# jqnfxa/Simplex-Method-Solver

Hardware: AMD Instinct MI355X
Metric: pivots/sec + achieved HBM GB/s, dense fp64 tableau, 1/2/4/8 MI355X (higher is better)
Workload: dtype f64; 1 GPU; 16384x16384 dense fp64 tableau, uniform random LP seed 0; rows=16384, cols=16384, n=16383, m=16383, parallelism=single GPU

## Files before the change

### simplex-method-solver_amd/csrc/smx_block.hpp

```cpp
#pragma once
#pragma clang fp contract(off)

namespace {

template <bool B>
struct SmxBool {
    static constexpr bool value = B;
};

constexpr int kBlkMax = 24;
constexpr int kBlkSlots = kBlkMax + 2;
constexpr int kBlkNT = kUpdBlock;
constexpr int kBlkScan = 4 * kBlkNT;
constexpr int kBlkPartsPer = kUpdBlock / kBlkNT;
constexpr int kBlkPartsMax = 4 * kMaxParts * kBlkPartsPer;
__host__ __device__ __forceinline__ int blk_parts_of(int nparts, int rows) {
    const int by_rows = (rows + kBlkNT - 1) / kBlkNT;
    int g = nparts * kBlkPartsPer;
    if (by_rows > g) g = by_rows;
    return g < kBlkPartsMax ? g : kBlkPartsMax;
}

struct BlkHdr {
    int32_t peff;
// ... 937 lines not shown
        int P, int parity, int bn, smx_ctl* __restrict__ ctl, BlkHdr* __restrict__ h,              \
        smx_part* __restrict__ parts, double* __restrict__ mul, double* __restrict__ pr,           \
        double* __restrict__ fr, const double* __restrict__ recv, int nranks,                      \
        int32_t* __restrict__ log, double* __restrict__ xhist, int64_t log_cap,                    \
        const double* __restrict__ xrow, int64_t xslot
#define SMX_BLK_STEP_ARGS                                                                           \
    T, ld, rows, m, flen, fscan, row0, P, parity, bn, ctl, h, parts, mul, pr, fr, recv, nranks,     \
        log, xhist, log_cap, xrow, xslot

template <int L, bool SH>
__global__ __launch_bounds__(kBlkNT) void k_blk_step(SMX_BLK_STEP_PARAMS) {
    blk_step_body<L, SH>(SMX_BLK_STEP_ARGS);
}

#undef SMX_BLK_STEP_PARAMS
#undef SMX_BLK_STEP_ARGS


template <int P, class PRS>
__device__ __forceinline__ dbl2 blk_exact_h(dbl2 v, int row, int j, const BlkHdr* __restrict__ h,
                                            const double* eq, PRS prs, const double* pc) {
#pragma unroll
    for (int q = 0; q < P; ++q) {
        const int rq = h->r[q], cq = h->c[q];
        const dbl2 p = prs(q);
#pragma unroll
        for (int hh = 0; hh < 2; ++hh) {
            const int jj = j + hh;
            double num;
            if (row == rq) {
                num = (jj == cq) ? 1.0 : -v[hh];
            } else {
                const double a = v[hh] * eq[q];
                const double b = p[hh] * pc[q];
                num = (jj == cq) ? v[hh] : (a - b);
            }
            v[hh] = num / eq[q];
        }
    }
    return v;
}

enum : int {
    kPcFast = 0,
    kPcZero,
    kPcWindow,
    kPcWindowFail,
    kPcExact,
    kPcChunkNotFree,
    kPcChunkNotZok,
    kPcRowFlag0,
    kPcRowFlag3,
    kPcXFail,
    kPcChunkE,
    kPcChunkP,
    kPcClkCycles,
    kPcClkTicks,
    kPcCount
};
#ifdef SMX_PATH_COUNT
__device__ unsigned long long g_path_cnt[kPcCount];
#define SMX_PC_DECL                                                                             \
    uint64_t pc_cnt[kPcCount] = {};                                                             \
    const uint64_t pc_t0 = __builtin_amdgcn_s_memtime();                                        \
    const uint64_t pc_r0 = __builtin_amdgcn_s_memrealtime();
#define SMX_PC(k) (++pc_cnt[(k)])
#define SMX_PC_FLUSH                                                                            \
    do {                                                                                        \
        pc_cnt[kPcClkCycles] = __builtin_amdgcn_s_memtime() - pc_t0;                            \
        pc_cnt[kPcClkTicks] = __builtin_amdgcn_s_memrealtime() - pc_r0;                         \
        const int l_ = threadIdx.x & (kWave - 1);                                               \
        uint64_t v_ = 0;                                                                        \
        _Pragma("unroll") for (int k_ = 0; k_ < kPcCount; ++k_) if (l_ == k_) v_ = pc_cnt[k_];  \
        if (l_ < kPcCount && v_) atomicAdd(&g_path_cnt[l_], (unsigned long long)v_);            \
    } while (0)
#else
#define SMX_PC_DECL
#define SMX_PC(k) ((void)0)
#define SMX_PC_FLUSH ((void)0)
#endif

__device__ int g_sweep_items = 16;

template <int P, int FORM>
__device__ __forceinline__ void blk_sweep_body_flag(const double* Tin, double* Tout, int64_t ld,
                                                    int R, int C, const BlkHdr* __restrict__ h,
                                                    const double* __restrict__ pr,
                                                    const double* __restrict__ mul) {
    constexpr bool LDS = FORM >= 5;
    constexpr bool ITEMS = FORM == 6;
    __shared__ dbl2 s_pr[LDS ? P : 1][kWave];
    __shared__ dbl2 s_ey[LDS ? P : 1];
    __shared__ dbl2 s_zm[LDS ? P : 1];
    __shared__ double s_zf;
    const int32_t* __restrict__ rfl = blk_rflags(mul, R);
    const int lane = threadIdx.x & (kWave - 1);
    const int wib = __builtin_amdgcn_readfirstlane(threadIdx.x >> 6);
    double eq[LDS ? 1 : P], yq[LDS ? 1 : P];
    bool allok = true;
#pragma unroll
    for (int q = 0; q < P; ++q) allok = allok && h->ok[q] != 0;
    constexpr int kChunk = 2 * kWave;
    const int nchunks = (C + kChunk - 1) / kChunk;
    int ch, base, qs;
    int c0 = 0, K = 1, stride = 1, seg = R;
    if constexpr (LDS) {
        ch = (int)blockIdx.x % nchunks;
        base = ((int)blockIdx.x / nchunks) * kUpdWaves + wib;
        qs = ((int)gridDim.x / nchunks) * kUpdWaves;
        if constexpr (ITEMS) {
            c0 = ch;
            K = max(1, min(g_sweep_items, nchunks));
            stride = max(1, nchunks / K);
            seg = ((R + K - 1) / K + qs - 1) / qs * qs;
        }
    } else {
        const int NW = (int)gridDim.x * kUpdWaves;
        const int w = (int)blockIdx.x * kUpdWaves + wib;
        ch = w % nchunks;
        base = w / nchunks;
        qs = NW / nchunks;
    }
    int j = ch * kChunk + 2 * lane;
    dbl2 prs[LDS ? 1 : P];
    auto stage = [&]() {
        for (int t = threadIdx.x; t < P * kWave; t += kUpdBlock) {
            const int q = t / kWave, jl = ch * kChunk + 2 * (t % kWave);
            s_pr[q][t % kWave] = jl < C ? *reinterpret_cast<const dbl2*>(pr + (int64_t)q * ld + jl)
                                        : dbl2{0.0, 0.0};
        }
    };
    if constexpr (LDS) {
        stage();
        if (threadIdx.x < P) {
            const int q = threadIdx.x;
            const double e = h->e[q];
            s_ey[q] = dbl2{e, h->y[q]};
            const double M = q == 0 ? e : (h->e[q - 1] < 0.0 ? e : -e);
            s_zm[q] = dbl2{M, fabs(h->y[q])};
            if (q == P - 1) s_zf = e < 0.0 ? 1.0 : -1.0;
        }
        __syncthreads();
    } else {
#pragma unroll
        for (int q = 0; q < P; ++q) {
            eq[q] = h->e[q];
            yq[q] = h->y[q];
            prs[q] = (j < C) ? *reinterpret_cast<const dbl2*>(pr + (int64_t)q * ld + j)
                             : dbl2{0.0, 0.0};
        }
    }
    auto PR = [&](int q) -> dbl2 {
        if constexpr (LDS) return s_pr[q][lane];
        else return prs[q];
    };
    auto EY = [&](int q) -> dbl2 {
        if constexpr (LDS) return s_ey[q];
        else return dbl2{eq[q], yq[q]};
    };
    const bool kNoFree = g_blk_nofree != 0;
    SMX_PC_DECL
    bool chunk_zok, chunk_free;
    auto chunk_flags = [&]() {
        uint32_t et = 0, pt = 0;
        bool zok = true;
#pragma unroll
        for (int q = 0; q < P; ++q) {
            const dbl2 p = PR(q);
            et = max(et, bnd_term(EY(q)[0]));
            if (j < C) {
                pt = max(pt, bnd_term(p[0]));
                zok = zok && bnd_or_zero(p[0]);
            }
// ... 75 lines not shown
                        const double tq = n[k] * y;
                        const double r = fma(-e, tq, n[k]);
                        rr[k] = fma(r, y, tq);
                    }
                    v0 = dbl2{rr[0], rr[1]};
                }
            }
            ok = true;
        } else if (chunk_zok && (rf & 1) && __all(bnd_or_zero(x0[0]) && bnd_or_zero(x0[1]))) {
            asm volatile("" ::: "memory");
            SMX_PC(kPcZero);
            if constexpr (!LDS) {
                dbl2 bq[P];
#pragma unroll
                for (int q = 0; q < P; ++q)
                    bq[q] = dbl2{prs[q][0] * pc0[q], prs[q][1] * pc0[q]};
#pragma unroll
                for (int q = 0; q < P; ++q) asm volatile("" : "+v"(bq[q]));
#pragma unroll
                for (int q = 0; q < P; ++q) {
                    const double e = eq[q], y = yq[q];
                    const double n0 = v0[0] * e - bq[q][0];
                    const double n1 = v0[1] * e - bq[q][1];
                    v0 = dbl2{fd_zero(n0, e, y), fd_zero(n1, e, y)};
                }
            } else {
#pragma unroll
                for (int q = 0; q < P && !SMX_ZNEG; ++q) {
                    const dbl2 p = PR(q);
                    const dbl2 ey = EY(q);
                    const double e = ey[0], y = ey[1];
                    double n[2];
                    n[0] = v0[0] * e - p[0] * pc0[q];
                    n[1] = v0[1] * e - p[1] * pc0[q];
                    v0 = dbl2{fd_zero(n[0], e, y), fd_zero(n[1], e, y)};
                }
#pragma unroll
                for (int q = 0; q < P && SMX_ZNEG; ++q) {
                    const dbl2 p = PR(q);
                    const dbl2 my = s_zm[q];
                    const double M = my[0], ya = my[1];
                    double n[2];
                    n[0] = v0[0] * M - p[0] * pc0[q];
                    n[1] = v0[1] * M - p[1] * pc0[q];
                    v0 = dbl2{fd_zneg(n[0], fabs(M), ya), fd_zneg(n[1], fabs(M), ya)};
                }
            }
            if (LDS && SMX_ZNEG) v0 = dbl2{v0[0] * s_zf, v0[1] * s_zf};
            ok = true;
        } else if (allok && rf != 2) {
            uint32_t wt = 0;
#pragma unroll
            for (int q = 0; q < P; ++q) {
                const dbl2 p = PR(q);
                const dbl2 ey = EY(q);
                const double e = ey[0], y = ey[1];
                double n[2];
                n[0] = v0[0] * e - p[0] * pc0[q];
                n[1] = v0[1] * e - p[1] * pc0[q];
                double rr[2];
#pragma unroll
                for (int k = 0; k < 2; ++k) {
                    const uint32_t tk = win_term(n[k]);
                    wt = max(wt, (dbits(n[k]) << 1) == 0 ? 0u : tk);
                    rr[k] = fd_zero(n[k], e, y);
                }
                v0 = dbl2{rr[0], rr[1]};
            }
            ok = __all(wt < kWinSpan);
            SMX_PC(ok ? kPcWindow : kPcWindowFail);
        } else {
            SMX_PC(kPcExact);
        }
        if (!ok) {
            x0 = ldc(i0);
            asm volatile("s_waitcnt vmcnt(0)" : "+v"(x0) :: "memory");
#pragma unroll
            for (int q = 0; q < P; ++q) eqa[q] = h->e[q];
            v0 = blk_exact_h<P>(x0, i0, j, h, eqa, PR, pc0);
        }
        if (j < C)
            __builtin_nontemporal_store(v0, reinterpret_cast<dbl2*>(Tout + (int64_t)i0 * ld + j));
    };
    if constexpr (!ITEMS) {
        if (base >= R) return;
    }
    for (int it = 0; it < K; ++it) {
        int lo = 0, hi = R;
        if constexpr (ITEMS) {
            lo = it * seg;
            hi = min(R, lo + seg);
            if (it > 0) {
                ch = (c0 + it * stride) % nchunks;
                j = ch * kChunk + 2 * lane;
                jc = min(j, (C - 1) & ~1);
                __syncthreads();
                stage();
                __syncthreads();
                chunk_flags();
            }
            if (lo + base >= hi) continue;
        }
        const int r0 = lo + base;
        dbl2 a = ldc(r0), b = ldc(r0 + qs);
        asm volatile("s_waitcnt vmcnt(1)" : "+v"(a) :: "memory");
        for (int i0 = r0; i0 < hi; i0 += 2 * qs) {
            rowf(a, i0);
            if (i0 + qs >= hi) break;
            a = ldc(i0 + 2 * qs);
            asm volatile("s_waitcnt vmcnt(2)" : "+v"(b) :: "memory");
            rowf(b, i0 + qs);
            if (i0 + 2 * qs >= hi) break;
            b = ldc(i0 + 3 * qs);
            asm volatile("s_waitcnt vmcnt(2)" : "+v"(a) :: "memory");
        }
        asm volatile("s_waitcnt vmcnt(0)" ::: "memory");
    }
    SMX_PC_FLUSH;
}

__device__ __forceinline__ void blk_fixcols(double* out, int64_t ld, int R, int P,
                                            const BlkHdr* __restrict__ h,
                                            const double* __restrict__ mul,
                                            const double* __restrict__ pr) {
    const double* mT = blk_mulT(mul, R);
    const int64_t pairs = (int64_t)R * P;
    for (int64_t t = (int64_t)blockIdx.x * kUpdBlock + threadIdx.x; t < pairs;
         t += (int64_t)gridDim.x * kUpdBlock) {
        const int q = (int)(t / R), i = (int)(t % R);
        const int c = h->c[q];
        bool last = true;
        for (int q2 = q + 1; q2 < P; ++q2) last = last && h->c[q2] != c;
        if (!last) continue;
        const double* mr = mul + (int64_t)i * kBlkMax;
        const bool frow = i == R - 1;
        double mq[kBlkMax], pc[kBlkMax], eq[kBlkMax];
        int rq[kBlkMax];
#pragma unroll
        for (int q2 = 0; q2 < kBlkMax; ++q2) {
            const bool act = q2 >= q && q2 < P;
            mq[q2] = act ? (frow ? mr[q2] : mT[(int64_t)q2 * R + i]) : 0.0;
            pc[q2] = (act && q2 > q) ? pr[(int64_t)q2 * ld + c] : 0.0;
            eq[q2] = act ? h->e[q2] : 1.0;
            rq[q2] = act ? h->r[q2] : -1;
        }
        double x = 0.0;
#pragma unroll
        for (int q2 = 0; q2 < kBlkMax; ++q2) {
            if (q2 < q || q2 >= P) continue;
            double num;
            if (q2 == q)
                num = (i == rq[q2]) ? 1.0 : mq[q2];
            else if (i == rq[q2])
                num = -x;
            else
                num = x * eq[q2] - pc[q2] * mq[q2];
            x = num / eq[q2];
        }
        out[(int64_t)i * ld + c] = x;
    }
}

__device__ __forceinline__ double* blk_out(double* b_in, double* b_other, int ipx, int in_idx,
                                           int applied, BlkHdr* __restrict__ hs) {
    const bool inplace = ipx >= 0 && ((ipx + applied) & 1) == 0;
    if (blockIdx.x == 0 && threadIdx.x == 0) hs->loc = inplace ? in_idx : in_idx ^ 1;
    return inplace ? b_in : b_other;
}

template <int P, int FORM>
__global__ __launch_bounds__(kUpdBlock) void k_blk_sweep(double* b_in, double* b_other, int64_t ld,
                                                         int R, int C,
                                                         const BlkHdr* __restrict__ h,
                                                         const double* __restrict__ mul,
                                                         const double* __restrict__ pr,
                                                         BlkHdr* __restrict__ hs, int ipx,
                                                         int in_idx) {
    if (h->peff != P) return;
    double* out = blk_out(b_in, b_other, ipx, in_idx, P, hs);
    blk_sweep_body_flag<P, FORM>(b_in, out, ld, R, C, h, pr, mul);
}

__device__ __forceinline__ void blk_publish_wave(const BlkHdr* __restrict__ h,
                                                 const smx_part* __restrict__ parts, int nparts,
                                                 int slot, int parity, smx_ctl* __restrict__ ctl) {
    if (ctl->term) return;
// ... 70 lines not shown
```

### simplex-method-solver_amd/csrc/smx_kernels.hip

```cpp
#include <hip/hip_runtime.h>

#include <math.h>
#include <stddef.h>
#include <stdint.h>
#include <stdio.h>
#include <stdlib.h>
#include <mutex>
#include <thread>
#include <vector>
#include <type_traits>
#include <utility>
#include <string.h>

#include <rccl/rccl.h>

#include "smx.h"

#pragma clang fp contract(off)

static_assert(sizeof(smx_ctl) == 128, "smx_ctl layout");
static_assert(offsetof(smx_ctl, term) == 16 && offsetof(smx_ctl, npivots) == 40 &&
                  offsetof(smx_ctl, shard_off) == 56 && offsetof(smx_ctl, xpos) == 64 &&
                  offsetof(smx_ctl, npiv) == 80 && offsetof(smx_ctl, dec) == 96,
              "smx_ctl offsets (mirrored in simplex_mi355x/_lib.py)");
// ... 307 lines not shown
                       reinterpret_cast<uint64_t*>(xch + p.row_off), s.ld, epoch,
                       g_resident_trace, g_resident_trace_from,
                       reinterpret_cast<uint64_t*>(xch + p.pc_off));
    return (int)hipGetLastError();
}

int resident_serialize(hipStream_t st, bool after) {
    static std::mutex mu;
    static hipEvent_t last[64] = {};
    int dev = 0;
    if (hipStreamGetDevice(st, &dev) != hipSuccess) (void)hipGetDevice(&dev);
    if (dev < 0 || dev >= 64) return (int)hipErrorInvalidDevice;
    std::lock_guard<std::mutex> lock(mu);
    if (!last[dev]) {
        int cur = 0;
        (void)hipGetDevice(&cur);
        hipError_t e = hipSetDevice(dev);
        if (e == hipSuccess) e = hipEventCreateWithFlags(&last[dev], hipEventDisableTiming);
        (void)hipSetDevice(cur);
        if (e != hipSuccess) return (int)e;
        if (!after) return 0;
    }
    return (int)(after ? hipEventRecord(last[dev], st) : hipStreamWaitEvent(st, last[dev], 0));
}

int launch_resident(double* buf0, double* buf1, const smx_shape& s, int parity, int k,
                    smx_ctl* ctl, void* xch, int64_t xch_bytes, uint32_t epoch, int32_t* log,
                    double* xhist, int64_t log_cap, hipStream_t st) {
    ResPlan p;
    if (!resident_plan(s, &p) || xch == nullptr || xch_bytes < p.bytes || epoch < 1 ||
        epoch > 4095 || k >= (1 << 20) - 1)
        return (int)hipErrorInvalidValue;
    hipError_t e = hipMemsetAsync(&ctl->dec[0][0], 0, sizeof(int32_t), st);
    if (e != hipSuccess) return (int)e;
    int err = resident_serialize(st, false);
    if (!err)
        err = launch_resident_kernel(buf0, buf1, s, p, parity, k, ctl, static_cast<char*>(xch),
                                     epoch, log, xhist, log_cap, st);
    if (!err) err = resident_serialize(st, true);
    return err;
}

int g_block = 0;
constexpr int64_t kBlockMinTable = 48ll << 20;
constexpr int64_t kBlockWideTable = 256ll << 20;

constexpr int64_t kBlockHugeTable = 1ll << 30;
bool wplan_shape(const smx_shape& s);

int block_pivots(const smx_shape& s) {
    if (g_block == 1) return 0;
    if (s.row0 != 0 || s.rows != s.n || s.rows < 1 || s.m < 1) return 0;
    if (g_block >= 2) return g_block;
    const int64_t bytes = (int64_t)(s.rows + 1) * s.ld * 8;
    if (bytes < kBlockMinTable) return 0;
    if (wplan_shape(s)) return kBlkMax;
    if (bytes >= kBlockHugeTable) return 20;
    return bytes >= kBlockWideTable ? 12 : 10;
}

int block_size(int k, int P, int b) {
    const int nb = (k + P - 1) / P;
    const int base = k / nb, extra = k % nb;
    return base + (b < extra ? 1 : 0);
}

using BlkSweepFn = void (*)(double*, double*, int64_t, int, int, const BlkHdr*, const double*,
                           const double*, BlkHdr*, int, int);
using BlkStepFn = void (*)(const double*, int64_t, int, int, int, int, int, int, int, int,
                           smx_ctl*, BlkHdr*, smx_part*, double*, double*, double*,
                           const double*, int, int32_t*, double*, int64_t, const double*,
                           int64_t);
using BshPackFn = void (*)(const double*, int64_t, int, int, int, int, int, const smx_ctl*,
                           const BlkHdr*, const smx_part*, int, const double*, const double*,
                           double*);

template <int FORM, int... Is>
BlkSweepFn blk_sweep_pick(int P, std::integer_sequence<int, Is...>) {
    static const BlkSweepFn t[] = {k_blk_sweep<Is + 1, FORM>...};
    return t[P - 1];
}
BlkSweepFn blk_sweep_fn(int P, int form) {
    using All = std::make_integer_sequence<int, kBlkMax>;
    return form == 6 ? blk_sweep_pick<6>(P, All{})
                     : form == 5 ? blk_sweep_pick<5>(P, All{}) : blk_sweep_pick<4>(P, All{});
}

template <bool SH, int... Is>
BlkStepFn blk_step_pick(int L, std::integer_sequence<int, Is...>) {
    static const BlkStepFn t[] = {k_blk_step<Is + 1, SH>...};
    return t[L - 1];
}
template <bool SH>
BlkStepFn blk_step_fn_sh(int L) {
    return blk_step_pick<SH>(L, std::make_integer_sequence<int, kBlkMax>{});
}

template <int... Is>
BshPackFn bsh_pack_pick(int D, std::integer_sequence<int, Is...>) {
    static const BshPackFn t[] = {k_bsh_pack<Is>...};
    return t[D];
}
BshPackFn bsh_pack_fn(int D) { return bsh_pack_pick(D, std::make_integer_sequence<int, kBlkMax>{}); }

struct BlkPtrs {
    BlkLayout L;
    BlkHdr* h[2];
    smx_part* parts;
    double *mul[2], *pr[2], *fr, *win;
    uint64_t* xg;
};
int g_block_planner = 0;
int g_block_nwin = kWin;
bool use_window(const smx_shape& s, bool sh) {
    return !sh && g_block_planner != 1 && s.row0 == 0 && s.rows == s.n;
}
bool use_wplan(const smx_shape& s, bool sh) {
    return use_window(s, sh) && g_block_planner == 0 && win_rpw(s.rows) <= kWpMaxRpw &&
           win_groups(s.rows) <= num_cus();
}
bool wplan_shape(const smx_shape& s) { return use_wplan(s, false); }

int blk_G(const smx_shape& s, bool sh) {
    return use_window(s, sh) ? win_groups(s.rows) : blk_parts_of(s.nparts, s.rows);
}

BlkPtrs blk_ptrs(const smx_shape& s, char* blk) {
    BlkPtrs b;
    b.L = blk_layout(s.rows + 1, s.ld, blk_parts_of(s.nparts, s.rows));
    for (int k = 0; k < 2; ++k) {
        b.h[k] = reinterpret_cast<BlkHdr*>(blk + kBlkHdrBytes * k);
        b.mul[k] = reinterpret_cast<double*>(blk + b.L.mul + k * b.L.mul_slot);
        b.pr[k] = reinterpret_cast<double*>(blk + b.L.pr + k * b.L.pr_slot);
    }
    b.parts = reinterpret_cast<smx_part*>(blk + b.L.parts);
    b.fr = reinterpret_cast<double*>(blk + b.L.fr);
    b.win = reinterpret_cast<double*>(blk + b.L.win);
    b.xg = reinterpret_cast<uint64_t*>(blk + b.L.xg);
    return b;
}

int launch_blk_prime(bool sh, const double* T, const smx_shape& s, int parity, int loc, smx_ctl* ctl,
                     const BlkPtrs& b, hipStream_t st) {
    hipLaunchKernelGGL(k_blk_start, dim3(blk_G(s, sh)), dim3(kBlkNT), 0, st, T, s.ld, s.rows, s.m,
                       fscan_of(s), parity, loc, s.row0, (const smx_ctl*)ctl, b.h[0], b.h[1],
                       b.fr, b.parts, use_wplan(s, sh) ? b.xg : nullptr);
    return (int)hipGetLastError();
}

int launch_blk_step(bool sh, int L, const double* T, const smx_shape& s, int P, int parity,
                    int bn, smx_ctl* ctl, const BlkPtrs& b, const double* recv, int nranks,
                    int32_t* log, double* xhist, int64_t log_cap, hipStream_t st,
                    const double* xrow = nullptr, int64_t xslot = 0) {
    BlkStepFn fn = sh ? blk_step_fn_sh<true>(L) : blk_step_fn_sh<false>(L);
    hipLaunchKernelGGL(fn, dim3(blk_G(s, sh)), dim3(kBlkNT), 0, st, T, s.ld, s.rows, s.m, s.flen,
                       fscan_of(s), s.row0, P, parity, bn, ctl, b.h[0], b.parts, b.mul[0],
                       b.pr[0], b.fr, recv, nranks, log, xhist, log_cap, xrow, xslot);
    return (int)hipGetLastError();
}

int launch_blk_wplan(const double* T, const smx_shape& s, int P, int parity, int bn, int done,
                     smx_ctl* ctl, const BlkPtrs& b, int32_t* log, double* xhist,
                     int64_t log_cap, hipStream_t st) {
    hipLaunchKernelGGL(k_blk_wplan, dim3(win_groups(s.rows)), dim3(kWinNT), 0, st, T, s.ld,
                       s.rows, s.m, s.flen, fscan_of(s), P, parity, bn, done, g_block_nwin,
                       win_rpw(s.rows), ctl, b.h[0], b.parts, b.mul[0], b.pr[0], b.xg, log,
                       xhist, log_cap);
    return (int)hipGetLastError();
}

int launch_blk_wstep(int L, const double* T, const smx_shape& s, int P, int parity, int bn,
                     smx_ctl* ctl, const BlkPtrs& b, int32_t* log, double* xhist, int64_t log_cap,
                     hipStream_t st, int fromT) {
    hipLaunchKernelGGL(k_blk_wstep, dim3(win_groups(s.rows)), dim3(kWinNT), 0, st, T, s.ld,
                       s.rows, s.m, s.flen, fscan_of(s), P, L, parity, bn, g_block_nwin,
                       win_rpw(s.rows), fromT, ctl, b.h[0], b.parts, b.mul[0], b.win, log, xhist,
                       log_cap);
    return (int)hipGetLastError();
}
int launch_blk_prows(const double* T, const smx_shape& s, int P, const BlkPtrs& b,
                     hipStream_t st) {
    const int64_t work = std::max<int64_t>((int64_t)(s.m + 1) * 4, s.rows + 1);
    const int grid = (int)std::min<int64_t>((work + kProwsNT - 1) / kProwsNT, num_cus() * 8);
    hipLaunchKernelGGL(k_blk_prows, dim3(grid), dim3(kProwsNT), 0, st, T, s.ld, s.rows, s.m, P,
                       (const BlkHdr*)b.h[0], b.mul[0], b.pr[0]);
    return (int)hipGetLastError();
}

int g_shard_xchg = -1;
bool xchg_light(int nranks) { return g_shard_xchg < 0 ? nranks >= 4 : g_shard_xchg == 1; }

int launch_bsh_pick(const double* hdrs, const smx_shape& s, int nranks, int rank,
                    const double* send, double* row, hipStream_t st) {
    const int grid = (int)((s.ld + kUpdBlock - 1) / kUpdBlock);
    hipLaunchKernelGGL(k_bsh_pick, dim3(grid < 1 ? 1 : grid), dim3(kUpdBlock), 0, st, hdrs,
                       nranks, s.ld, s.m, s.flen, rank, send, row);
    return (int)hipGetLastError();
}

int launch_bsh_pack(int D, const double* T, const smx_shape& s, int P, int bn,
                    const smx_ctl* ctl, const BlkPtrs& b, double* send, hipStream_t st) {
    const int gc = (int)std::min<int64_t>((s.m + 1 + kBlkNT - 1) / kBlkNT, kBlkPartsMax);
    const int grid = std::max(blk_parts_of(s.nparts, s.rows), gc);
    hipLaunchKernelGGL(bsh_pack_fn(D), dim3(grid), dim3(kBlkNT), 0, st, T, s.ld, s.rows,
                       s.m, s.row0, P, bn, ctl, (const BlkHdr*)b.h[0], (const smx_part*)b.parts,
                       blk_parts_of(s.nparts, s.rows), (const double*)b.mul[0], (const double*)b.pr[0], send);
    return (int)hipGetLastError();
}

int launch_blk_publish(bool sh, const smx_shape& s, int parity, int bn, smx_ctl* ctl, const BlkPtrs& b,
                       hipStream_t st) {
    hipLaunchKernelGGL(k_blk_publish, dim3(1), dim3(kWave), 0, st, (const BlkHdr*)b.h[0],
                       (const smx_part*)b.parts, blk_G(s, sh), blk_slot(0, 1, bn), parity, ctl);
    return (int)hipGetLastError();
}

int g_block_form = 0;
constexpr int kSweepRegMaxP = 12;
constexpr int64_t kSweepItemRows = 2048;

int sweep_grid_lds(const smx_shape& s, int bpc) {
    const int64_t nchunks = (s.m + 1 + 2 * kWave - 1) / (2 * kWave);
    int64_t per = (int64_t)num_cus() * bpc / nchunks;
    const int64_t rows_per = (s.rows + 1 + kUpdWaves - 1) / kUpdWaves;
    if (per > rows_per) per = rows_per;
    if (per < 1) per = 1;
    return (int)(per * nchunks);
}

int launch_block_sweep(bool sh, double* tin, double* tother, const smx_shape& s, int P, char* blk,
                       const BlkLayout& L, hipStream_t st, int slot = 0, int ipx = 0,
                       int in_idx = 0, int ipx_part = 0, smx_ctl* pub_ctl = nullptr,
                       int pub_bn = 0, int pub_parity = 0) {
    const int nchunks = (s.m + 1 + 2 * kWave - 1) / (2 * kWave);
    int form = g_block_form >= 4 && g_block_form <= 6 ? g_block_form
                                                      : (P > kSweepRegMaxP ? 5 : 4);
    int grid = 0;
    if (form == 4) {
        grid = update_grid(s, (const void*)blk_sweep_fn(P, 4), 0, 5);
        if (((int64_t)grid * kUpdWaves) % nchunks != 0) form = 5;
    }
    if (form == 5 && g_block_form == 0) {
        const int64_t per = sweep_grid_lds(s, g_blocks_per_cu > 0 ? g_blocks_per_cu : 8) / nchunks;
        if ((int64_t)(s.rows + 1) >= per * kUpdWaves * kSweepItemRows) form = 6;
    }
    BlkSweepFn fn = blk_sweep_fn(P, form);
    if (form >= 5)
        grid = sweep_grid_lds(s, g_blocks_per_cu > 0 ? g_blocks_per_cu : 8);
    BlkHdr* hs = reinterpret_cast<BlkHdr*>(blk);
    const BlkHdr* h = reinterpret_cast<const BlkHdr*>(blk + kBlkHdrBytes * slot);
    const double* mul = reinterpret_cast<const double*>(blk + L.mul + slot * L.mul_slot);
    const double* pr = reinterpret_cast<const double*>(blk + L.pr + slot * L.pr_slot);
    hipLaunchKernelGGL(fn, dim3(grid), dim3(kUpdBlock), 0, st, tin, tother, s.ld, s.rows + 1,
                       s.m + 1, h, mul, pr, hs, ipx, in_idx);
    const int64_t fix_wg = ((int64_t)(s.rows + 1) * P + kUpdBlock - 1) / kUpdBlock;
    const int rest_grid = (int)std::max<int64_t>(num_cus() * 2,
                                                 std::min<int64_t>(fix_wg, num_cus() * 8));
    hipLaunchKernelGGL(k_blk_sweep_rest, dim3(rest_grid), dim3(kUpdBlock), 0, st, tin,
                       tother, s.ld, s.rows + 1, s.m + 1, P, h, mul, pr, hs, ipx_part, in_idx, 1,
                       ipx, reinterpret_cast<const smx_part*>(blk + L.parts), blk_G(s, sh),
                       blk_slot(0, 1, pub_bn), pub_parity, pub_ctl);
    return (int)hipGetLastError();
}


int launch_block_chain(double* buf0, double* buf1, const smx_shape& s, int parity, int k, int P,
                       smx_ctl* ctl, char* blk, int32_t* log, double* xhist, int64_t log_cap,
                       hipStream_t st, hipEvent_t* ev = nullptr, double* send = nullptr,
                       double* recv = nullptr, int nranks = 0, ncclComm_t comm = nullptr) {
    const BlkPtrs bp = blk_ptrs(s, blk);
    const bool sh = comm != nullptr;
    const size_t slot = (size_t)SMX_SHARD_HDR + 2 * (size_t)s.ld;
    const bool light = sh && xchg_light(nranks);
    int rank = 0;
    if (light && ncclCommUserRank(comm, &rank) != ncclSuccess) return (int)hipErrorInvalidValue;
    double* xrow = light ? recv + (size_t)nranks * SMX_SHARD_HDR : nullptr;
    int err = launch_blk_prime(sh, parity ? buf1 : buf0, s, parity, parity, ctl, bp, st);
    int p = parity, done = 0, bn = 0;
    while (!err && done < k) {
        const int Pb = block_size(k, P, bn);
        double* tin = p ? buf1 : buf0;
        double* toth = p ? buf0 : buf1;
        const bool wplan = use_wplan(s, sh);
        if (!err && wplan)
            err = launch_blk_wplan(tin, s, Pb, p, bn, done, ctl, bp, log, xhist, log_cap, st);
        for (int l = 1; l <= Pb && !err && !wplan; ++l) {
            if (sh) {
                err = launch_bsh_pack(l - 1, tin, s, Pb, bn, ctl, bp, send, st);
                if (!err && !light) {
                    const ncclResult_t r = ncclAllGather(send, recv, slot, ncclFloat64, comm, st);
                    if (r != ncclSuccess) err = -1000 - (int)r;
                } else if (!err) {
                    ncclResult_t r = ncclAllGather(send, recv, SMX_SHARD_HDR, ncclFloat64, comm, st);
                    if (r == ncclSuccess) {
                        err = launch_bsh_pick(recv, s, nranks, rank, send, xrow, st);
                        if (!err)
                            r = ncclAllReduce(xrow, xrow, (size_t)s.ld, ncclInt64, ncclMax, comm,
                                              st);
                    }
                    if (r != ncclSuccess) err = -1000 - (int)r;
                }
            }
            if (!err && use_window(s, sh))
                err = launch_blk_wstep(l, tin, s, Pb, p, bn, ctl, bp, log, xhist, log_cap, st,
                                       bn == 0 && l == 1);
            else if (!err)
                err = launch_blk_step(sh, l, tin, s, Pb, p, bn, ctl, bp, recv, nranks, log,
                                      xhist, log_cap, st, xrow,
                                      light ? (int64_t)SMX_SHARD_HDR : 0);
#ifdef SMX_BLK_TRACE_TWICE
            if (!err && !sh)
                err = launch_blk_step(sh, l, tin, s, Pb, p, bn, ctl, bp, recv, nranks, log,
                                      xhist, log_cap, st, xrow, 0);
#endif
        }
        if (!err && use_window(s, sh) && !(wplan && wp_inpr(s.m + 1, win_groups(s.rows))))
            err = launch_blk_prows(tin, s, Pb, bp, st);
        if (ev) (void)hipEventRecord(ev[2 * bn], st);
        const bool lastb = done + Pb >= k;
        if (!err)
            err = launch_block_sweep(sh, tin, toth, s, Pb, blk, bp.L, st, 0, 0, p, 0,
                                     lastb ? ctl : nullptr, bn + 1, (p + Pb) & 1);
        if (ev) (void)hipEventRecord(ev[2 * bn + 1], st);
        p = (p + Pb) & 1;
        done += Pb;
        ++bn;
    }
// ... 729 lines not shown
    if (workgroups >= -1) g_resident = workgroups > kResBlock ? kResBlock : workgroups;
    return prev;
}

int64_t smx_tune_resident_timeout(int64_t ticks) {
    int64_t prev = -1;
    if (hipMemcpyFromSymbol(&prev, HIP_SYMBOL(g_res_spin_ticks), sizeof prev) != hipSuccess)
        return -1;
    if (ticks >= 0 &&
        hipMemcpyToSymbol(HIP_SYMBOL(g_res_spin_ticks), &ticks, sizeof ticks) != hipSuccess)
        return -1;
    return prev;
}

int smx_resident_trace(void* trace, int32_t from_step) {
    g_resident_trace = static_cast<uint64_t*>(trace);
    g_resident_trace_from = from_step < 0 ? 0 : from_step;
    return 0;
}

int64_t smx_resident_bytes(const smx_shape* shape, int32_t* plan_out) {
    ResPlan p;
    if (!shape_ok(shape) || !resident_plan(*shape, &p)) return 0;
    if (plan_out) {
        plan_out[0] = p.G;
        plan_out[1] = p.rpw;
        plan_out[2] = p.ept;
        plan_out[3] = (int32_t)p.lds;
    }
    return p.bytes;
}

int smx_resident_run(double* buf0, double* buf1, const smx_shape* shape, int32_t parity,
                     int32_t k, smx_ctl* ctl, void* xch, int64_t xch_bytes, int32_t epoch,
                     int32_t* log, double* xhist, int64_t log_cap, void* stream) {
    if (!shape_ok(shape) || buf0 == buf1 || k < 0) return (int)hipErrorInvalidValue;
    return launch_resident(buf0, buf1, *shape, parity & 1, k, ctl, xch, xch_bytes,
                           (uint32_t)epoch, log, xhist, log_cap, S(stream));
}

int smx_fastdiv_check(const double* num, const double* den, int64_t count,
                      unsigned long long* out, void* stream) {
    if (count < 0 || !num || !den || !out) return (int)hipErrorInvalidValue;
    hipError_t e = hipMemsetAsync(out, 0, 2 * sizeof(unsigned long long), S(stream));
    if (e != hipSuccess) return (int)e;
    hipLaunchKernelGGL(k_fastdiv_check, dim3(1024), dim3(256), 0, S(stream), num, den, count,
                       out);
    return (int)hipGetLastError();
}

int smx_fastdiv_check_bounded(const double* num, const double* den, int64_t count,
                              unsigned long long* out, void* stream) {
    if (count < 0 || !num || !den || !out) return (int)hipErrorInvalidValue;
    hipError_t e = hipMemsetAsync(out, 0, 4 * sizeof(unsigned long long), S(stream));
    if (e != hipSuccess) return (int)e;
    hipLaunchKernelGGL(k_fastdiv_bounded_check, dim3(1024), dim3(256), 0, S(stream), num, den,
                       count, out);
    return (int)hipGetLastError();
}

int smx_diag_path_counts(int64_t* out, int32_t count, int32_t clear) {
#ifdef SMX_PATH_COUNT
    if (!out || count < 0) return (int)hipErrorInvalidValue;
    unsigned long long v[kPcCount];
    hipError_t e = hipDeviceSynchronize();
    if (e == hipSuccess) e = hipMemcpyFromSymbol(v, HIP_SYMBOL(g_path_cnt), sizeof v);
    if (e != hipSuccess) return (int)e;
    for (int k = 0; k < count && k < kPcCount; ++k) out[k] = (int64_t)v[k];
    if (clear) {
        static const unsigned long long zero[kPcCount] = {};
        e = hipMemcpyToSymbol(HIP_SYMBOL(g_path_cnt), zero, sizeof zero);
    }
    return e == hipSuccess ? kPcCount : (int)e;
#else
    (void)out;
    (void)count;
    (void)clear;
    return -(int)hipErrorNotSupported;
#endif
}

int smx_tune_block_form(int32_t form) {
    const int prev = g_block_form;
    if (form == 0 || (form >= 4 && form <= 6)) g_block_form = form;
    return prev;
}

int smx_tune_block_planner(int32_t planner, int32_t nwin) {
    const int prev = g_block_planner;
    if (planner >= 0 && planner <= 2) g_block_planner = planner;
    if (nwin >= 2 && nwin <= kWin) g_block_nwin = nwin;
    else if (nwin == 0) g_block_nwin = kWin;
    return prev;
}

int smx_tune_block(int32_t pivots) {
    const int prev = g_block;
    if (pivots >= 0) g_block = pivots > kBlkMax ? kBlkMax : pivots;
    return prev;
}

int64_t smx_block_bytes(const smx_shape* shape, int32_t* pivots_inout) {
    static const int nofree_env = [] {
        const char* e = getenv("SMX_BLK_NOFREE");
        const int v = (e && e[0] == '1') ? 1 : 0;
        if (v) (void)hipMemcpyToSymbol(HIP_SYMBOL(g_blk_nofree), &v, sizeof v);
        const char* it = getenv("SMX_SWEEP_ITEMS");
        const int k = it ? atoi(it) : 0;
        if (k > 0) (void)hipMemcpyToSymbol(HIP_SYMBOL(g_sweep_items), &k, sizeof k);
        return v;
    }();
    (void)nofree_env;
    if (!shape_ok(shape)) return 0;
    const int req = pivots_inout ? *pivots_inout : 0;
    if (req < 0 || req > kBlkMax) return 0;
    const int P = req > 0 ? req : block_pivots(*shape);
    if (P < 1 || !block_args_ok(shape, 0, P, shape, INT64_MAX)) return 0;
    if (pivots_inout) *pivots_inout = P;
    return blk_layout(shape->rows + 1, shape->ld, blk_parts_of(shape->nparts, shape->rows)).bytes;
}

int smx_block_run(double* buf0, double* buf1, const smx_shape* shape, int32_t parity, int32_t k,
                  int32_t pivots, smx_ctl* ctl, void* blk, int64_t blk_bytes, int32_t* log,
                  double* xhist, int64_t log_cap, void* stream) {
    if (!block_chain_ok(shape, k, pivots, blk, blk_bytes, buf0, buf1, ctl))
        return (int)hipErrorInvalidValue;
    if (k == 0) return 0;
    return launch_block_chain(buf0, buf1, *shape, parity & 1, k, pivots, ctl,
                              static_cast<char*>(blk), log, xhist, log_cap, S(stream));
}

int smx_block_run_timed(double* buf0, double* buf1, const smx_shape* shape, int32_t parity,
                        int32_t k, int32_t pivots, smx_ctl* ctl, void* blk, int64_t blk_bytes,
                        int32_t* log, double* xhist, int64_t log_cap, void* stream,
                        float* host_sweep_ms, float* host_total_ms) {
    const bool defer = !host_sweep_ms && !host_total_ms;
    if (!block_chain_ok(shape, k, pivots, blk, blk_bytes, buf0, buf1, ctl) || k < 1 ||
        (!defer && (!host_sweep_ms || !host_total_ms)))
        return (int)hipErrorInvalidValue;
    const int nb = (k + pivots - 1) / pivots;
    const int err = run_timed(S(stream), nb, true, host_sweep_ms, host_total_ms,
                              [&](hipEvent_t* ev) {
        return launch_block_chain(buf0, buf1, *shape, parity & 1, k, pivots, ctl,
                                  static_cast<char*>(blk), log, xhist, log_cap, S(stream), ev);
    });
    if (defer && !err) g_timed_blocks = nb;
    return err;
}

int smx_block_timed_read(int32_t blocks, float* host_sweep_ms, float* host_total_ms) {
    if (blocks < 1 || blocks != g_timed_blocks || !host_sweep_ms || !host_total_ms)
        return (int)hipErrorInvalidValue;
    g_timed_blocks = 0;
    return timed_read(blocks, true, host_sweep_ms, host_total_ms);
}

int smx_block_graph_create(double* buf0, double* buf1, const smx_shape* shape, int32_t parity,
                           int32_t k, int32_t pivots, smx_ctl* ctl, void* blk, int64_t blk_bytes,
                           int32_t* log, double* xhist, int64_t log_cap, void* stream,
                           void** graph_out) {
    if (!block_chain_ok(shape, k, pivots, blk, blk_bytes, buf0, buf1, ctl) || k < 1 ||
        !graph_out)
        return (int)hipErrorInvalidValue;
    return capture_graph(S(stream), graph_out, [&] {
        return launch_block_chain(buf0, buf1, *shape, parity & 1, k, pivots, ctl,
                                  static_cast<char*>(blk), log, xhist, log_cap, S(stream));
    });
// ... 422 lines not shown
```

Measured before the change: 12880 pivots/s.

## Add paired-row sweep form that processes two rows per step with phased multiplier loads

Adds a new block-sweep form (7) that handles two tableau rows per iteration. Each pivot column's LDS pivot-row value and eta are loaded once and applied to both rows, and the per-row multipliers are loaded in phases of 12 into scalar registers. The form is selected automatically when the block has at least 20 pivots and enough rows per wave. It aims to cut LDS reads and raise arithmetic per load in the memory-bound update. In exchange it raises register pressure and adds a deeper four-load prefetch pipeline, with a fallback to the per-row path when the fast conditions fail.

```diff
diff --git a/simplex-method-solver_amd/csrc/smx_block.hpp b/simplex-method-solver_amd/csrc/smx_block.hpp
--- a/simplex-method-solver_amd/csrc/smx_block.hpp
+++ b/simplex-method-solver_amd/csrc/smx_block.hpp
@@ -1043,6 +1043,27 @@
 
 __device__ int g_sweep_items = 16;
 
+constexpr int kPairPhase = 12;
+
+__device__ __forceinline__ void blk_pair_step(dbl2& va, dbl2& vb, dbl2 p, dbl2 ey, double ma,
+                                              double mb) {
+    const double e = ey[0], y = ey[1];
+    double n[4];
+    n[0] = va[0] * e - p[0] * ma;
+    n[1] = va[1] * e - p[1] * ma;
+    n[2] = vb[0] * e - p[0] * mb;
+    n[3] = vb[1] * e - p[1] * mb;
+    double rr[4];
+#pragma unroll
+    for (int k = 0; k < 4; ++k) {
+        const double tq = n[k] * y;
+        const double r = fma(-e, tq, n[k]);
+        rr[k] = fma(r, y, tq);
+    }
+    va = dbl2{rr[0], rr[1]};
+    vb = dbl2{rr[2], rr[3]};
+}
+
 template <int P, int FORM>
 __device__ __forceinline__ void blk_sweep_body_flag(const double* Tin, double* Tout, int64_t ld,
                                                     int R, int C, const BlkHdr* __restrict__ h,
@@ -1050,6 +1071,7 @@
                                                     const double* __restrict__ mul) {
     constexpr bool LDS = FORM >= 5;
     constexpr bool ITEMS = FORM == 6;
+    constexpr bool PAIRS = FORM == 7;
     __shared__ dbl2 s_pr[LDS ? P : 1][kWave];
     __shared__ dbl2 s_ey[LDS ? P : 1];
     __shared__ dbl2 s_zm[LDS ? P : 1];
@@ -1291,6 +1313,58 @@
         if (j < C)
             __builtin_nontemporal_store(v0, reinterpret_cast<dbl2*>(Tout + (int64_t)i0 * ld + j));
     };
+    auto pairf = [&](dbl2 xa, dbl2 xb, int ia, int hi) {
+        constexpr int NPH = (P + kPairPhase - 1) / kPairPhase;
+        constexpr int P0 = P < kPairPhase ? P : kPairPhase;
+        const int ib = ia + qs;
+        const bool two = ib < hi;
+        const int ibc = two ? ib : ia;
+        const double* ma = mul + (int64_t)ia * kBlkMax;
+        const double* mb = mul + (int64_t)ibc * kBlkMax;
+        int rfa = rfl[ia], rfb = rfl[ibc];
+        asm volatile("" : "+s"(rfa));
+        asm volatile("" : "+s"(rfb));
+        const uint32_t xt = max(max((uint32_t)__double2hiint(xa[0]) << 1,
+                                    (uint32_t)__double2hiint(xa[1]) << 1),
+                                max((uint32_t)__double2hiint(xb[0]) << 1,
+                                    (uint32_t)__double2hiint(xb[1]) << 1));
+        if (two && chunk_free && rfa == 1 && rfb == 1 && __all(xt < kBndXMax)) {
+            SMX_PC(kPcFast);
+            SMX_PC(kPcFast);
+            dbl2 va = xa, vb = xb;
+            double pa[P0], pb[P0];
+#pragma unroll
+            for (int ph = 0; ph < NPH; ++ph) {
+                const int q0 = ph * kPairPhase;
+                const int nq = P - q0 < kPairPhase ? P - q0 : kPairPhase;
+                int o = q0;
+                asm volatile("" : "+s"(o) : "v"(va), "v"(vb));
+#pragma unroll
+                for (int q = 0; q < nq; ++q) {
+                    pa[q] = ma[o + q];
+                    pb[q] = mb[o + q];
+                }
+#pragma unroll
+                for (int q = 0; q < nq; ++q) {
+                    asm volatile("" : "+s"(pa[q]));
+                    asm volatile("" : "+s"(pb[q]));
+                }
+#pragma unroll
+                for (int q = 0; q < nq; ++q)
+                    blk_pair_step(va, vb, s_pr[q0 + q][lane], s_ey[q0 + q], pa[q], pb[q]);
+            }
+            asm volatile("" : "+v"(va), "+v"(vb));
+            if (j < C) {
+                __builtin_nontemporal_store(va,
+                                            reinterpret_cast<dbl2*>(Tout + (int64_t)ia * ld + j));
+                __builtin_nontemporal_store(vb,
+                                            reinterpret_cast<dbl2*>(Tout + (int64_t)ib * ld + j));
+            }
+        } else {
+#pragma nounroll
+            for (int s = 0; s < (two ? 2 : 1); ++s) rowf(s ? xb : xa, s ? ib : ia);
+        }
+    };
     if constexpr (!ITEMS) {
         if (base >= R) return;
     }
@@ -1311,6 +1385,28 @@
             if (lo + base >= hi) continue;
         }
         const int r0 = lo + base;
+        if constexpr (PAIRS) {
+            int i0 = r0;
+            dbl2 a0 = ldc(i0), a1 = ldc(i0 + qs);
+            dbl2 b0 = ldc(i0 + 2 * qs), b1 = ldc(i0 + 3 * qs);
+            asm volatile("s_waitcnt vmcnt(2)" : "+v"(a0), "+v"(a1) :: "memory");
+            for (;;) {
+                pairf(a0, a1, i0, hi);
+                i0 += 2 * qs;
+                if (i0 >= hi) break;
+                a0 = ldc(i0 + 2 * qs);
+                a1 = ldc(i0 + 3 * qs);
+                asm volatile("s_waitcnt vmcnt(4)" : "+v"(b0), "+v"(b1) :: "memory");
+                pairf(b0, b1, i0, hi);
+                i0 += 2 * qs;
+                if (i0 >= hi) break;
+                b0 = ldc(i0 + 2 * qs);
+                b1 = ldc(i0 + 3 * qs);
+                asm volatile("s_waitcnt vmcnt(4)" : "+v"(a0), "+v"(a1) :: "memory");
+            }
+            asm volatile("s_waitcnt vmcnt(0)" ::: "memory");
+            continue;
+        }
         dbl2 a = ldc(r0), b = ldc(r0 + qs);
         asm volatile("s_waitcnt vmcnt(1)" : "+v"(a) :: "memory");
         for (int i0 = r0; i0 < hi; i0 += 2 * qs) {
diff --git a/simplex-method-solver_amd/csrc/smx_kernels.hip b/simplex-method-solver_amd/csrc/smx_kernels.hip
--- a/simplex-method-solver_amd/csrc/smx_kernels.hip
+++ b/simplex-method-solver_amd/csrc/smx_kernels.hip
@@ -413,7 +413,8 @@
 }
 BlkSweepFn blk_sweep_fn(int P, int form) {
     using All = std::make_integer_sequence<int, kBlkMax>;
-    return form == 6 ? blk_sweep_pick<6>(P, All{})
+    return form == 7 ? blk_sweep_pick<7>(P, All{})
+           : form == 6 ? blk_sweep_pick<6>(P, All{})
                      : form == 5 ? blk_sweep_pick<5>(P, All{}) : blk_sweep_pick<4>(P, All{});
 }
 
@@ -549,6 +550,8 @@
 int g_block_form = 0;
 constexpr int kSweepRegMaxP = 12;
 constexpr int64_t kSweepItemRows = 2048;
+constexpr int kSweepPairMinP = 20;
+constexpr int64_t kSweepPairRows = 64;
 
 int sweep_grid_lds(const smx_shape& s, int bpc) {
     const int64_t nchunks = (s.m + 1 + 2 * kWave - 1) / (2 * kWave);
@@ -564,7 +567,7 @@
                        int in_idx = 0, int ipx_part = 0, smx_ctl* pub_ctl = nullptr,
                        int pub_bn = 0, int pub_parity = 0) {
     const int nchunks = (s.m + 1 + 2 * kWave - 1) / (2 * kWave);
-    int form = g_block_form >= 4 && g_block_form <= 6 ? g_block_form
+    int form = g_block_form >= 4 && g_block_form <= 7 ? g_block_form
                                                       : (P > kSweepRegMaxP ? 5 : 4);
     int grid = 0;
     if (form == 4) {
@@ -574,6 +577,8 @@
     if (form == 5 && g_block_form == 0) {
         const int64_t per = sweep_grid_lds(s, g_blocks_per_cu > 0 ? g_blocks_per_cu : 8) / nchunks;
         if ((int64_t)(s.rows + 1) >= per * kUpdWaves * kSweepItemRows) form = 6;
+        else if (P >= kSweepPairMinP && (int64_t)(s.rows + 1) >= per * kUpdWaves * kSweepPairRows)
+            form = 7;
     }
     BlkSweepFn fn = blk_sweep_fn(P, form);
     if (form >= 5)
@@ -1469,7 +1474,7 @@
 
 int smx_tune_block_form(int32_t form) {
     const int prev = g_block_form;
-    if (form == 0 || (form >= 4 && form <= 6)) g_block_form = form;
+    if (form == 0 || (form >= 4 && form <= 7)) g_block_form = form;
     return prev;
 }
 
```

After: 13430 pivots/s, median of 6. +4.2%, better.
